# moddyz/stereo-to-multiview-cuda

Hardware: AMD Instinct MI355X
Metric: stereo->8-view frames/sec @1080p d=64; cost-agg HBM GB/s vs roofline (higher is better)
Workload: dtype f32; 1 GPU; 1920x1080 synthetic stereo frame, D=64, zd=32, full stereo->8-view frame: cost init + cross aggregation + WTA + DCC/IRV x5/bilateral + 6 DIBR views + interlacing, one frame per GPU per step; stages=3, usd=34, lsd=17, views=8, aggregation=matrix pipe (stm_kernels_aggm.hip)

## Files before the change

### include/stm_hip.h

```cpp
#ifndef STM_HIP_H
#define STM_HIP_H

#ifdef __cplusplus
extern "C" {
#endif
#if defined(STM_BUILD) && defined(__GNUC__)
#pragma GCC visibility push(default)
#endif

int         stm_version(void);
void        stm_set_stream(void *hip_stream);
void       *stm_get_stream(void);
void        stm_set_error_mode(int mode);
const char *stm_last_error(void);
void        stm_release_workspace(void);
void        stm_prof_enable(int on);
void        stm_prof_reset(void);
int         stm_prof_read(const char *kernel, float *total_ms);
void        stm_set_agg_variant(int v);
int         stm_agg_path(int num_disp, int zero_disp, int num_rows, int num_cols, int usd, int stages);
int         stm_first_pass_path(int num_disp, int zero_disp, int num_rows, int num_cols, int usd, int stages);
int         stm_px_order(int num_disp, int zero_disp, int num_rows, int num_cols, int usd, int stages);
void        stm_set_irv_paper_ratio(int on);
int         stm_set_irv_chunk(int entries);
int         stm_irv_path(int num_rows, int num_cols, int usd, int iterations, int device_flavour, int with_dcc);
int         stm_set_lens(int mode, double pitch, double slope, double centre);
int         stm_set_depth(int mode, float gain, float conv);
int         stm_set_depth_auto(float disp_lo, float disp_hi, float max_gain, int clip_permille, float rate, float *d_state);
int         stm_set_antialias(int mode, float strength, int max_radius, float gate);
void        stm_get_antialias(int out_mode[2], float out[2]);
int         stm_set_align(int mode, float a, float b, float c);
int         stm_set_align_auto(int radius, float rate, float *d_state);
void        stm_get_align(int out_mode[2], float out[4]);
int         stm_set_balance(int mode, const unsigned char *lut768);
int         stm_set_balance_auto(int max_shift, float rate, int *d_state);
void        stm_get_balance(int out_mode[2], float *out_rate, unsigned char out_lut[768]);
int         stm_set_cut(int mode, int thresh_permille, int min_gap, int *d_state);
void        stm_get_cut(int out[3]);
int         stm_set_active(int mode, const int rect[4], int fill, float fill_disp);
int         stm_set_active_auto(int thresh_luma, int lit_permille, int max_bar_permille, int hold, int *d_state);
void        stm_get_active(int out[10], float *fill_disp);
int         stm_set_layout(int layout, int tiles_x, int tiles_y, int order, int filter);
void        stm_get_layout(int *out);
int         stm_set_output(int format, int matrix, int pitch, int uv_row);
void        stm_get_output(int out[4]);
int         stm_set_overlay(int mode, const unsigned char *d_overlay, int ov_rows, int ov_cols, int x0, int y0, float disparity);
void        stm_get_overlay(int out[5], float *disparity);
int         stm_set_overlay_auto(int mode, int near_permille, float margin, int pad, float limit_lo, float limit_hi, float rate_near,
// ... 43 lines not shown
void stm_d_dr_irv(float *d_disp, unsigned char *d_outliers, unsigned char **d_cross, int thresh_s, float thresh_h,
                  int num_rows, int num_cols, int num_disp, int zero_disp, int usd, int iterations);
void stm_dr_interp(float *disp, unsigned char *outliers, unsigned char *img, int num_rows, int num_cols, int elem_sz);
void stm_d_dr_interp(float *d_disp, unsigned char *d_outliers, unsigned char *d_img, int num_rows, int num_cols, int elem_sz);
void stm_filter_bilateral_1(float *img, int radius, float sigma_color, float sigma_spatial,
                            int num_rows, int num_cols, int num_disp);
void stm_d_filter_bilateral_1(float *d_img, int radius, float sigma_color, float sigma_spatial,
                              int num_rows, int num_cols, int num_disp);
void stm_filter_gaussian_1(float *img, int radius, float sigma_spatial, int num_rows, int num_cols);
void stm_d_filter_gaussian_1(float *d_img, int radius, float sigma_spatial, int num_rows, int num_cols);
void stm_filter_bleed_1(unsigned char *img, int radius, int num_rows, int num_cols);
void stm_d_filter_bleed_1(unsigned char *d_img, int radius, int num_rows, int num_cols);
void stm_filter_median(float *img, int num_rows, int num_cols);
void stm_d_filter_median(float *d_img, int num_rows, int num_cols);

void stm_dibr_occl(unsigned char *occl_l, unsigned char *occl_r, float *disp_l, float *disp_r,
                   int num_rows, int num_cols);
void stm_d_dibr_occl(unsigned char *d_occl_l, unsigned char *d_occl_r, float *d_disp_l, float *d_disp_r,
                     int num_rows, int num_cols);
void stm_dibr_occl_to_mask(float *mask_l, float *mask_r, unsigned char *occl_l, unsigned char *occl_r,
                           int num_rows, int num_cols);
void stm_d_dibr_occl_to_mask(float *d_mask_l, float *d_mask_r, unsigned char *d_occl_l, unsigned char *d_occl_r,
                             int num_rows, int num_cols);
void stm_dibr_dbm(unsigned char *img_out, unsigned char *img_in_l, unsigned char *img_in_r,
                  float *disp_l, float *disp_r, unsigned char *occl_l, unsigned char *occl_r,
                  float *mask_l, float *mask_r, float shift, int num_rows, int num_cols, int elem_sz);
void stm_d_dibr_dbm(unsigned char *d_img_out, unsigned char *d_img_in_l, unsigned char *d_img_in_r,
                    float *d_disp_l, float *d_disp_r, unsigned char *d_occl_l, unsigned char *d_occl_r,
                    float *d_mask_l, float *d_mask_r, float shift, int num_rows, int num_cols, int elem_sz);
void stm_dibr_dbm_lin(unsigned char *img_out, unsigned char *img_in_l, unsigned char *img_in_r,
                      float *disp_l, float *disp_r, unsigned char *occl_l, unsigned char *occl_r,
                      float *mask_l, float *mask_r, float shift, int num_rows, int num_cols, int elem_sz);
void stm_d_dibr_dbm_lin(unsigned char *d_img_out, unsigned char *d_img_in_l, unsigned char *d_img_in_r,
                        float *d_disp_l, float *d_disp_r, unsigned char *d_occl_l, unsigned char *d_occl_r,
                        float *d_mask_l, float *d_mask_r, float shift, int num_rows, int num_cols, int elem_sz);
void stm_dibr_dfm(unsigned char *img_out, unsigned char *img_in_l, unsigned char *img_in_r,
                  float *disp_l, float *disp_r, float shift, int num_rows, int num_cols, int elem_sz);
void stm_d_dibr_dfm(unsigned char *d_img_out, unsigned char *d_img_in_l, unsigned char *d_img_in_r,
                    float *d_disp_l, float *d_disp_r, float shift, int num_rows, int num_cols, int elem_sz);

void stm_mux_multiview(unsigned char **views, unsigned char *out_data, int num_views, float angle,
                       int in_rows, int in_cols, int out_rows, int out_cols, int elem_sz);
void stm_d_mux_multiview(unsigned char **d_views, unsigned char *d_out_data, int num_views, float angle,
                         int in_rows, int in_cols, int out_rows, int out_cols, int elem_sz);
void stm_mux_multiview_lens(unsigned char **views, unsigned char *out_data, int num_views, int mode, double pitch, double slope,
                            double centre, int in_rows, int in_cols, int out_rows, int out_cols, int elem_sz);
// ... 231 lines not shown
```

### stereo-to-multiview-cuda_amd/_lib.py

```python
import ctypes as C
import os

HERE = os.path.dirname(os.path.abspath(__file__))
LIB_PATH = os.path.join(HERE, "libstm_hip.so")
if os.environ.get("STM_LIB") == "timing":
    LIB_PATH = os.path.join(HERE, "libstm_hip_timing.so")

u8p = C.POINTER(C.c_uint8)
f32p = C.POINTER(C.c_float)
u32p = C.POINTER(C.c_uint32)
u8pp = C.POINTER(u8p)
f32pp = C.POINTER(f32p)
vp = C.c_void_p
i, f, d = C.c_int, C.c_float, C.c_double

PROTOS = {
    "stm_version": ([], i),
    "stm_set_stream": ([vp], None),
    "stm_get_stream": ([], vp),
    "stm_set_error_mode": ([i], None),
    "stm_last_error": ([], C.c_char_p),
    "stm_release_workspace": ([], None),
    "stm_prof_enable": ([i], None),
    "stm_prof_reset": ([], None),
    "stm_prof_read": ([C.c_char_p, f32p], i),
    "stm_set_agg_variant": ([i], None),
    "stm_agg_path": ([i, i, i, i, i, i], i),
    "stm_first_pass_path": ([i, i, i, i, i, i], i),
    "stm_px_order": ([i, i, i, i, i, i], i),
    "stm_set_irv_paper_ratio": ([i], None),
    "stm_set_irv_chunk": ([i], i),
    "stm_irv_path": ([i, i, i, i, i, i], i),
    "stm_set_ref_quirks": ([i], None),
    "stm_set_lens": ([i, d, d, d], i),
    "stm_set_layout": ([i, i, i, i, i], i),
    "stm_get_layout": ([C.POINTER(C.c_int)], None),
    "stm_set_output": ([i, i, i, i], i),
    "stm_get_output": ([C.POINTER(C.c_int)], None),
    "stm_set_overlay": ([i, vp, i, i, i, i, f], i),
    "stm_get_overlay": ([C.POINTER(C.c_int), f32p], None),
    "stm_set_overlay_auto": ([i, i, f, i, f, f, f, f, vp], i),
    "stm_get_overlay_auto": ([C.POINTER(C.c_int), f32p], None),
    "stm_set_quilt_lds_limit": ([i], None),
    "stm_set_packing": ([i, i, i, i], i),
    "stm_get_packing": ([C.POINTER(C.c_int)], None),
    "stm_set_depth": ([i, f, f], i),
    "stm_set_depth_auto": ([f, f, f, i, f, vp], i),
    "stm_set_antialias": ([i, f, i, f], i),
    "stm_get_antialias": ([C.POINTER(C.c_int), f32p], None),
    "stm_set_align": ([i, f, f, f], i),
    "stm_set_align_auto": ([i, f, vp], i),
    "stm_get_align": ([C.POINTER(C.c_int), f32p], None),
    "stm_set_balance": ([i, u8p], i),
    "stm_set_balance_auto": ([i, f, vp], i),
    "stm_get_balance": ([C.POINTER(C.c_int), f32p, u8p], None),
# ... 11 lines not shown
    "stm_dc_subpixel": ([f32pp, f32p, i, i, i, i], None),
    "stm_d_dc_subpixel": ([vp, vp, i, i, i, i], None),
    "stm_dc_hslo": ([f32pp, f32p, u8p, u8p, f, f, f, i, i, i, i, i], None),
    "stm_d_dc_hslo": ([vp, vp, vp, vp, f, f, f, i, i, i, i, i], None),
    "stm_dr_dcc": ([u8p, u8p, f32p, f32p, i, i], None),
    "stm_d_dr_dcc": ([vp, vp, vp, vp, i, i], None),
    "stm_dr_irv": ([f32p, u8p, u8pp, i, f, i, i, i, i, i, i], None),
    "stm_d_dr_irv": ([vp, vp, vp, i, f, i, i, i, i, i, i], None),
    "stm_dr_interp": ([f32p, u8p, u8p, i, i, i], None),
    "stm_d_dr_interp": ([vp, vp, vp, i, i, i], None),
    "stm_filter_bilateral_1": ([f32p, i, f, f, i, i, i], None),
    "stm_d_filter_bilateral_1": ([vp, i, f, f, i, i, i], None),
    "stm_filter_gaussian_1": ([f32p, i, f, i, i], None),
    "stm_d_filter_gaussian_1": ([vp, i, f, i, i], None),
    "stm_filter_bleed_1": ([u8p, i, i, i], None),
    "stm_d_filter_bleed_1": ([vp, i, i, i], None),
    "stm_filter_median": ([f32p, i, i], None),
    "stm_generate_gaussian_kernel": ([f32p, i, f], None),
    "stm_d_filter_median": ([vp, i, i], None),
    "stm_dibr_occl": ([u8p, u8p, f32p, f32p, i, i], None),
    "stm_d_dibr_occl": ([vp, vp, vp, vp, i, i], None),
    "stm_dibr_occl_to_mask": ([f32p, f32p, u8p, u8p, i, i], None),
    "stm_d_dibr_occl_to_mask": ([vp, vp, vp, vp, i, i], None),
    "stm_dibr_dbm": ([u8p, u8p, u8p, f32p, f32p, u8p, u8p, f32p, f32p, f, i, i, i], None),
    "stm_d_dibr_dbm": ([vp, vp, vp, vp, vp, vp, vp, vp, vp, f, i, i, i], None),
    "stm_dibr_dbm_lin": ([u8p, u8p, u8p, f32p, f32p, u8p, u8p, f32p, f32p, f, i, i, i], None),
    "stm_d_dibr_dbm_lin": ([vp, vp, vp, vp, vp, vp, vp, vp, vp, f, i, i, i], None),
    "stm_dibr_dfm": ([u8p, u8p, u8p, f32p, f32p, f, i, i, i], None),
    "stm_d_dibr_dfm": ([vp, vp, vp, vp, vp, f, i, i, i], None),
    "stm_mux_multiview": ([u8pp, u8p, i, f, i, i, i, i, i], None),
    "stm_d_mux_multiview": ([vp, vp, i, f, i, i, i, i, i], None),
    "stm_mux_multiview_lens": ([u8pp, u8p, i, i, d, d, d, i, i, i, i, i], None),
    "stm_d_mux_multiview_lens": ([vp, vp, i, i, d, d, d, i, i, i, i, i], None),
    "stm_quilt_multiview": ([u8pp, u8p, i, i, i, i, i, i, i, i, i, i], None),
    "stm_d_quilt_multiview": ([vp, vp, i, i, i, i, i, i, i, i, i, i], None),
    "stm_mux_overlay": ([u8p, u8p, i, i, i, i, f, i, f, i, d, d, d, i, i, i, i, i, i, i], None),
    "stm_d_mux_overlay": ([vp, vp, i, i, i, i, f, i, f, i, d, d, d, i, i, i, i, i, i, i], None),
    "stm_d_demux_sbs": ([vp, vp, vp, i, i, i, i], None),
    "stm_demux_nv12": ([u8p, u8p, u8p, i, u8p, i, i, i, i, i, i], None),
    "stm_d_demux_nv12": ([vp, vp, vp, i, vp, i, i, i, i, i, i], None),
    "stm_mux_nv12": ([u8p, i, u8p, i, u8p, i, i, i, i], None),
    "stm_d_mux_nv12": ([vp, i, vp, i, vp, i, i, i, i], None),
    "stm_demux_packed": ([u8p, u8p, u8p, i, i, i, i, i, i, i, i], None),
    "stm_d_demux_packed": ([vp, vp, vp, i, i, i, i, i, i, i, i], None),
    "stm_demux_nv12_packed": ([u8p, u8p, u8p, i, u8p, i, i, i, i, i, i, i, i, i, i], None),
    "stm_d_demux_nv12_packed": ([vp, vp, vp, i, vp, i, i, i, i, i, i, i, i, i, i], None),
# ... 101 lines not shown
```

### stereo-to-multiview-cuda_amd/csrc/stm_api.hip

```cpp
#include "stm_common.h"
#include <initializer_list>
#include <mutex>
#include "../../include/stm_hip.h"

#include <map>
#include <stdio.h>
#include <stdlib.h>
#include <string.h>
#include <tuple>
#include <vector>

using namespace stm;

namespace {

struct DevTable {
    float *d = nullptr;
    size_t n = 0;
};
std::map<std::tuple<int, int, float, float>, DevTable> g_tables;

int cur_dev()
{
    int dev = 0;
// ... 154 lines not shown
Arms arms_from_table(unsigned char **d_cross)
{
    u8 *h[4];
    STM_CHECK(hipMemcpyAsync(h, d_cross, sizeof h, hipMemcpyDeviceToHost, stream()));
    sync();
    return Arms{h[0], h[1], h[2], h[3]};
}

void core_bilateral(float *d_img, int radius, float sigma_color, float sigma_spatial, int H, int W, int D)
{
    size_t HW = (size_t)H * W;
    float *tmp = Workspace::get<float>(HW);
    launch_bilateral(d_img, tmp, gauss2d_table(radius, sigma_spatial), gauss1d_table(D, sigma_color), radius, H, W, D);
    STM_CHECK(hipMemcpyAsync(d_img, tmp, HW * sizeof(float), hipMemcpyDeviceToDevice, stream()));
}

void core_dbm(u8 *d_out, const u8 *d_l, const u8 *d_r, const float *disp_l, const float *disp_r, const float *mask_l,
              const float *mask_r, float shift, int H, int W, int elem_sz, int g_radius, float g_sigma, bool linear = false)
{
    size_t HW = (size_t)H * W;
    float *blend = Workspace::get<float>(HW);
    launch_gaussian_max(mask_r, blend, gauss2d_table(g_radius, g_sigma), g_radius, g_sigma, H, W, true);
    launch_view_synth(d_out, d_l, d_r, disp_l, disp_r, mask_l, mask_r, blend, shift, H, W, elem_sz, linear);
}

void dbm_device(const char *fn, unsigned char *d_img_out, unsigned char *d_img_in_l, unsigned char *d_img_in_r, float *d_disp_l,
                float *d_disp_r, float *d_mask_l, float *d_mask_r, float shift, int num_rows, int num_cols, int elem_sz, bool linear)
{
    if (!args_ok(fn, {{"num_rows", num_rows, 1}, {"num_cols", num_cols, 1}, {"elem_sz", elem_sz, 3}})) return;
    Workspace::begin((size_t)num_rows * num_cols * 4 + 1024);
    if (elem_sz > 3)
        STM_CHECK(hipMemsetAsync(d_img_out, 0, (size_t)num_rows * num_cols * elem_sz, stream()));
    core_dbm(d_img_out, d_img_in_l, d_img_in_r, d_disp_l, d_disp_r, d_mask_l, d_mask_r, shift, num_rows, num_cols, elem_sz,
             10, 15.0f, linear);
}
void dbm_host(const char *fn, unsigned char *img_out, unsigned char *img_in_l, unsigned char *img_in_r, float *disp_l, float *disp_r,
              float *mask_l, float *mask_r, float shift, int num_rows, int num_cols, int elem_sz, bool linear)
{
    if (!args_ok(fn, {{"num_rows", num_rows, 1}, {"num_cols", num_cols, 1}, {"elem_sz", elem_sz, 3}})) return;
    size_t HW = (size_t)num_rows * num_cols;
    Workspace::begin(3 * HW * elem_sz + 20 * HW + 8192);
    u8 *l = up(img_in_l, HW * elem_sz), *r = up(img_in_r, HW * elem_sz), *o = Workspace::get<u8>(HW * elem_sz);
    float *dl = up(disp_l, HW), *dr = up(disp_r, HW), *ml = up(mask_l, HW), *mr = up(mask_r, HW);
    STM_CHECK(hipMemsetAsync(o, 0, HW * elem_sz, stream()));
    core_dbm(o, l, r, dl, dr, ml, mr, shift, num_rows, num_cols, elem_sz, 7, 10.0f, linear);
    down(img_out, o, HW * elem_sz);
// ... 527 lines not shown
                     int num_cols)
{
    if (!args_ok("d_dibr_occl", {{"num_rows", num_rows, 1}, {"num_cols", num_cols, 1}})) return;
    launch_occl(d_occl_l, d_occl_r, d_disp_l, d_disp_r, num_rows, num_cols);
}
void stm_dibr_occl(unsigned char *occl_l, unsigned char *occl_r, float *disp_l, float *disp_r, int num_rows, int num_cols)
{
    if (!args_ok("dibr_occl", {{"num_rows", num_rows, 1}, {"num_cols", num_cols, 1}})) return;
    size_t HW = (size_t)num_rows * num_cols;
    Workspace::begin(10 * HW + 4096);
    float *dl = up(disp_l, HW), *dr = up(disp_r, HW);
    u8 *ol = Workspace::get<u8>(HW), *orr = Workspace::get<u8>(HW);
    launch_occl(ol, orr, dl, dr, num_rows, num_cols);
    down(occl_l, ol, HW); down(occl_r, orr, HW);
    sync();
}

void stm_d_dibr_occl_to_mask(float *d_mask_l, float *d_mask_r, unsigned char *d_occl_l, unsigned char *d_occl_r,
                             int num_rows, int num_cols)
{
    if (!args_ok("d_dibr_occl_to_mask", {{"num_rows", num_rows, 1}, {"num_cols", num_cols, 1}})) return;
    launch_occl_to_mask(d_mask_l, d_mask_r, d_occl_l, d_occl_r, num_rows, num_cols);
}
void stm_dibr_occl_to_mask(float *mask_l, float *mask_r, unsigned char *occl_l, unsigned char *occl_r, int num_rows,
                           int num_cols)
{
    if (!args_ok("dibr_occl_to_mask", {{"num_rows", num_rows, 1}, {"num_cols", num_cols, 1}})) return;
    size_t HW = (size_t)num_rows * num_cols;
    Workspace::begin(10 * HW + 4096);
    u8 *ol = up(occl_l, HW), *orr = up(occl_r, HW);
    float *ml = Workspace::get<float>(HW), *mr = Workspace::get<float>(HW);
    launch_occl_to_mask(ml, mr, ol, orr, num_rows, num_cols);
    down(mask_l, ml, HW); down(mask_r, mr, HW);
    sync();
}

void stm_d_dibr_dbm(unsigned char *d_img_out, unsigned char *d_img_in_l, unsigned char *d_img_in_r, float *d_disp_l,
                    float *d_disp_r, unsigned char *d_occl_l, unsigned char *d_occl_r, float *d_mask_l, float *d_mask_r,
                    float shift, int num_rows, int num_cols, int elem_sz)
{
    (void)d_occl_l; (void)d_occl_r;
    dbm_device("d_dibr_dbm", d_img_out, d_img_in_l, d_img_in_r, d_disp_l, d_disp_r, d_mask_l, d_mask_r, shift, num_rows, num_cols,
               elem_sz, false);
}
void stm_dibr_dbm(unsigned char *img_out, unsigned char *img_in_l, unsigned char *img_in_r, float *disp_l, float *disp_r,
                  unsigned char *occl_l, unsigned char *occl_r, float *mask_l, float *mask_r, float shift, int num_rows,
// ... 1061 lines not shown
        if (!overlay_tiles_ok(fn, lo, num_views)) return false;
        if (overlay_auto().mode == 1 && !overlay_fit_size_ok(fn, a.num_rows, a.num_cols)) return false;
    }
    if (lo.layout == 0) return frame_output_ok(fn, lo, Hout, Wout);
    if (lens().mode != 0) {
        char msg[200];
        snprintf(msg, sizeof msg, "%s: layout 1 (quilt) together with lens mode %d: a quilt is not interlaced, set one of them to 0", fn, lens().mode);
        fail(msg, "layout, lens", __FILE__, __LINE__);
        return false;
    }
    return quilt_args_ok(fn, lo, num_views, a.num_rows, a.num_cols, Hout, Wout, "num_views", "num_rows_out", "num_cols_out") &&
           frame_output_ok(fn, lo, Hout, Wout);
}

void frame_render(u8 *img_l, u8 *img_r, float *d_disp_l, float *d_disp_r, u8 *d_interlaced, const FrameArgs &a, float **depth_state_out,
                  const int *d_rect)
{
    *depth_state_out = nullptr;
    const int H = a.num_rows, W = a.num_cols, Hout = a.num_rows_out, Wout = a.num_cols_out, elem_sz = a.elem_sz, N = a.num_views;
    const float angle = a.angle;
    const bool linear = (a.stages & 0x800) != 0;
    const size_t HW = (size_t)H * W, IMG = HW * elem_sz;
    float *mask_l = Workspace::get<float>(HW), *mask_r = Workspace::get<float>(HW), *blend = Workspace::get<float>(HW);
    launch_hitmask_rows(mask_l, mask_r, d_disp_l, d_disp_r, H, W);
    launch_gaussian_max(mask_r, blend, gauss2d_table(10, 15.0f), 10, 15.0f, H, W, true);

    const Lens ln = lens();
    const Depth dp = depth();
    const Layout lo = layout();
    float inv_y = 0.0f;
    int ymod = 1;
    if (lo.layout == 0 && dp.mode != 0 && ln.mode == 0 && !mux_geom_ok(N, angle, elem_sz, nullptr, &inv_y, &ymod)) return;
    float *state = nullptr;
    if (dp.mode == 2) {
        uint32_t *hist = Workspace::get<uint32_t>(4096);
        state = dp.d_state ? dp.d_state : Workspace::get<float>(4);
        launch_depth_fit(state, hist, d_disp_l, d_disp_r, H, W, dp.disp_lo, dp.disp_hi, dp.max_gain, dp.clip_permille, dp.rate,
                         dp.d_state == nullptr, d_rect);
        *depth_state_out = state;
    }
    const Antialias aa = antialias();
    if (aa.mode == 1) {
        u8 *flt[2] = {Workspace::get<u8>(IMG), Workspace::get<u8>(IMG)};
        const u8 *src[2] = {img_l, img_r};
        const float *dsp[2] = {d_disp_l, d_disp_r};
        launch_view_prefilter(2, flt, src, dsp, H, W, elem_sz, N, aa.strength, aa.max_radius, aa.gate, dp.mode == 1 ? dp.gain : 1.0f,
                              dp.mode == 1 ? dp.conv : 0.0f, state);
        img_l = flt[0];
// ... 814 lines not shown
```

### stereo-to-multiview-cuda_amd/csrc/stm_common.h

```cpp
#pragma once
#include <hip/hip_runtime.h>
#include <stddef.h>
#include <stdint.h>

typedef unsigned char u8;

namespace stm {

void fail(const char *what, const char *expr, const char *file, int line);
bool failed();
void clear_failed();
struct ApiNest { ApiNest(); ~ApiNest(); };
bool api_outermost();
void release_host_frame_bufs();
bool nv12_args_ok(const char *fn, int num_rows, int num_cols_sbs, int num_cols, const char *cols_name, int pitch_y, int pitch_uv, int matrix);
#define STM_CHECK(expr)                                                                  \
    do {                                                                                 \
        hipError_t _e = (expr);                                                          \
        if (_e != hipSuccess) ::stm::fail(hipGetErrorString(_e), #expr, __FILE__, __LINE__); \
    } while (0)
#define STM_CHECK_LAUNCH() STM_CHECK(hipGetLastError())
#define STM_LAUNCH(...)                                     \
    do {                                                    \
        if (!::stm::failed()) hipLaunchKernelGGL(__VA_ARGS__); \
// ... 183 lines not shown
void launch_dcc(u8 *out_l, u8 *out_r, const float *disp_l, const float *disp_r, u8 *hit_l, u8 *hit_r, int H, int W);
void launch_irv(int nviews, float *const *disp, u8 *const *outl, const u8 *const *up, const u8 *const *down,
                const u8 *const *left, const u8 *const *right, int thresh_s, float thresh_h,
                int H, int W, int D, int zd, int usd, int iterations, bool device_flavour, bool with_dcc = false);
int irv_path(int H, int W, int usd, int iterations, bool device_flavour, bool with_dcc);
void launch_bilateral(const float *in, float *out, const float *spatial, const float *color,
                      int radius, int H, int W, int D);
void launch_bilateral2(const float *in_a, float *out_a, const float *in_b, float *out_b, const float *spatial, const float *color,
                       int radius, int H, int W, int D, bool integer_maps = false, const float *one_value = nullptr, int zd = 0);
void launch_gaussian_max(const float *in, float *out, const float *spatial, int radius, float sigma, int H, int W,
                         bool invert_input);
void launch_subpix(Vol cost, float *disp, int D, int zd, int H, int W);
void launch_subpix_frame(float *const *pq, float *const *quads, float *const *disp, const u8 *const *armL, const u8 *const *armR, int D,
                         int zd, int H, int W);
void launch_interp(int nviews, float *const *disp, const u8 *const *outl, const u8 *const *img, int H, int W, int elem_sz);
void launch_demux_sbs(u8 *l, u8 *r, const u8 *sbs, int H, int Wsbs, int W, int elem_sz);
void launch_demux_sbs_packed(u8 *l, u8 *r, uint32_t *pk_l, uint32_t *pk_r, uint32_t *wide_l, uint32_t *wide_r, const u8 *sbs, int H,
                             int Wsbs, int W, int elem_sz);
void launch_occl(u8 *occl_l, u8 *occl_r, const float *disp_l, const float *disp_r, int H, int W);
void launch_bleed(const u8 *in, u8 *out, int radius, int H, int W);
void launch_median3(const float *in, float *out, int H, int W);
void launch_dcc_rows(u8 *out_l, u8 *out_r, const float *disp_l, const float *disp_r, int H, int W);
void launch_hitmask_rows(float *mask_l, float *mask_r, const float *disp_l, const float *disp_r, int H, int W);
void launch_occl_to_mask(float *mask_l, float *mask_r, const u8 *occl_l, const u8 *occl_r, int H, int W);
void launch_view_synth(u8 *out, const u8 *img_l, const u8 *img_r, const float *disp_l, const float *disp_r,
                       const float *mask_l, const float *mask_r, const float *blend, float shift, int H, int W, int elem_sz,
                       bool linear = false);
void launch_view_synth_all(u8 *views, size_t view_stride, int N, const u8 *img_l, const u8 *img_r, const float *disp_l,
                           const float *disp_r, const float *mask_l, const float *mask_r, const float *blend, int H, int W,
                           int elem_sz, bool linear = false);
void launch_fwarp(u8 *out, const u8 *img, const float *disp, float shift, unsigned long long *keys, int H, int W, int elem_sz);
void launch_scale_bilinear(const u8 *in, u8 *out, int in_rows, int in_cols, int out_rows, int out_cols, int elem_sz);
void launch_disp_scale(float *out, const float *in, int out_rows, int out_cols, int in_rows, int in_cols, float disp_scale);
void launch_view_table(u8 **tab, u8 *first, u8 *last, u8 *mem, size_t stride, int N);
void launch_disp_upsample(int nviews, float *const *out, const float *const *dlow, const u8 *const *ilow, const u8 *const *img,
                          const float *tab, int H, int W, int h, int w, int elem_sz, float up);
void launch_disp_temporal(int nviews, float *const *cur, const float *const *prev, const u8 *const *img, const u8 *const *img_prev,
                          const size_t *byte_off, int H, int W, int stride, int elem_sz, float alpha, int thresh_color, float thresh_disp);
void launch_synth_mux(const u8 *img_l, const u8 *img_r, const float *disp_l, const float *disp_r, const float *mask_l, const float *mask_r,
                      const float *blend, u8 *out, int N, float y_interval, float inv_y_interval, int ymod, int Hin, int Win, int Hout,
                      int Wout, int elem_sz, int variant, bool linear = false);
void launch_mux(const u8 *const *d_views, u8 *out, int N, float y_interval, float inv_y_interval, int ymod,
                int Hin, int Win, int Hout, int Wout, int elem_sz, int variant);
void launch_mux_lens(const u8 *const *d_views, u8 *out, int N, const Lens &ln, int Hin, int Win, int Hout, int Wout, int elem_sz);
void launch_synth_mux_lens(const u8 *img_l, const u8 *img_r, const float *disp_l, const float *disp_r, const float *mask_l,
                           const float *mask_r, const float *blend, u8 *out, int N, const Lens &ln, int Hin, int Win, int Hout, int Wout,
// ... 172 lines not shown
```

### stereo-to-multiview-cuda_amd/csrc/stm_kernels_dibr.hip

```cpp
#include "stm_common.h"
#include "stm_views.h"

namespace stm {

__global__ __launch_bounds__(256) void stm_k_demux_sbs(u8 *__restrict__ l, u8 *__restrict__ r, const u8 *__restrict__ sbs,
                                                       int H, int Wsbs, int W, int elem_sz)
{
    int x = blockIdx.x * 256 + threadIdx.x, y = blockIdx.y;
    if (x >= Wsbs) return;
    const u8 *s = sbs + ((size_t)y * Wsbs + x) * elem_sz;
    u8 *d;
    if (x < W) d = l + ((size_t)y * W + x) * elem_sz;
    else if (x - W < W) d = r + ((size_t)y * W + (x - W)) * elem_sz;
    else return;
    d[0] = s[0]; d[1] = s[1]; d[2] = s[2];
}
__global__ __launch_bounds__(256) void stm_k_demux_sbs_packed(u8 *__restrict__ l, u8 *__restrict__ r, uint32_t *__restrict__ pk_l,
                                                              uint32_t *__restrict__ pk_r, uint32_t *__restrict__ wide_l,
                                                              uint32_t *__restrict__ wide_r, const u8 *__restrict__ sbs, int Wsbs,
                                                              int W, int elem_sz)
{
    const int x = blockIdx.x * 256 + threadIdx.x, y = blockIdx.y;
    if (x >= 2 * W) return;
    const u8 *s = sbs + ((size_t)y * Wsbs + x) * elem_sz;
// ... 142 lines not shown
    __syncthreads();
    const size_t orow = (size_t)ty * W;
    for (int tx = threadIdx.x; tx < W; tx += 256) {
        int cnt_l = 0, cnt_r = 0;
#pragma unroll
        for (int j = 0; j < 3; ++j) {
            const u8 *ol = hm_lds + (size_t)j * 2 * W, *orr = ol + W;
#pragma unroll
            for (int x = -1; x <= 1; ++x) {
                int sx = tx + x;
                if (sx < 0) sx = -sx;
                if (sx > W - 1) sx = W - 1 - x;
                sx = min(max(sx, 0), W - 1);
                cnt_l += ol[sx] > 0;
                cnt_r += orr[sx] > 0;
            }
        }
        const u8 vl = ((double)cnt_l > 8 * 0.30) ? (u8)1 : hm_lds[2 * W + tx];
        const u8 vr = ((double)cnt_r > 8 * 0.30) ? (u8)1 : hm_lds[3 * W + tx];
        mask_l[orow + tx] = vl == 1 ? 1.0f : 0.0f;
        mask_r[orow + tx] = vr == 1 ? 1.0f : 0.0f;
    }
}
void launch_hitmask_rows(float *mask_l, float *mask_r, const float *disp_l, const float *disp_r, int H, int W)
{
    const size_t smem = 6 * (size_t)W;
    if (smem > 64 * 1024) STM_CHECK(hipFuncSetAttribute((const void *)stm_k_hitmask_rows, hipFuncAttributeMaxDynamicSharedMemorySize, (int)smem));
    STM_LAUNCH(stm_k_hitmask_rows, dim3(H), dim3(256), smem, stream(), mask_l, mask_r, disp_l, disp_r, H, W);
    STM_CHECK_LAUNCH();
}

template <bool LINEAR>
__device__ __forceinline__ u8 warp_tap(const u8 *__restrict__ img, size_t row, float fx, int c, int W, int elem_sz)
{
    if constexpr (!LINEAR) {
        const int sx = (int)fx;
        return img[(row + sx) * elem_sz + c];
    } else {
        const int x0 = (int)floorf(fx);
        const int x1 = min(x0 + 1, W - 1);
        const float wx = fx - (float)x0;
        const float a = (float)img[(row + x0) * elem_sz + c] * (1.0f - wx);
        const float b = (float)img[(row + x1) * elem_sz + c] * wx;
        const float top = a + b;
        return (u8)top;
    }
}
template <bool LINEAR>
__global__ __launch_bounds__(256) void stm_k_view_synth(u8 *__restrict__ out, const u8 *__restrict__ img_l,
                                                        const u8 *__restrict__ img_r, const float *__restrict__ disp_l,
                                                        const float *__restrict__ disp_r, const float *__restrict__ mask_l,
// ... 275 lines not shown
    ta = top * (1.0f - wy);
    tb = bot * wy;
    return (u8)(ta + tb);
}
template <bool LINEAR>
__global__ __launch_bounds__(256) void stm_k_synth_mux(SynthArgs a, u8 *__restrict__ out, int N, float y_interval, float inv_y, int ymod,
                                                       int Hin, int Win, int Hout, int Wout, int elem_sz, int variant)
{
    const int tx = blockIdx.x * 256 + threadIdx.x, ty = blockIdx.y;
    if (tx >= Wout) return;
    float xs = ((float)tx / (float)Wout) * (float)Win;
    xs = fminf(fmaxf(xs, 0.0f), (float)(Win - 1));
    float ys = ((float)ty / (float)Hout) * (float)Hin;
    ys = fminf(fmaxf(ys, 0.0f), (float)(Hin - 1));
    const int r_view = mux_r_view(tx, ty, N, y_interval, inv_y, ymod, variant);
    int g_view = r_view + 1, b_view = r_view + 2;
    if (g_view >= N) g_view -= N;
    if (b_view >= N) b_view -= N;
    const size_t o = ((size_t)tx + (size_t)ty * Wout) * elem_sz;
    out[o + 0] = synth_bilinear<LINEAR>(a, N, b_view, 0, xs, ys, Win, Hin, elem_sz);
    out[o + 1] = synth_bilinear<LINEAR>(a, N, g_view, 1, xs, ys, Win, Hin, elem_sz);
    out[o + 2] = synth_bilinear<LINEAR>(a, N, r_view, 2, xs, ys, Win, Hin, elem_sz);
}
void launch_synth_mux(const u8 *img_l, const u8 *img_r, const float *disp_l, const float *disp_r, const float *mask_l, const float *mask_r,
                      const float *blend, u8 *out, int N, float y_interval, float inv_y_interval, int ymod, int Hin, int Win, int Hout,
                      int Wout, int elem_sz, int variant, bool linear)
{
    SynthArgs a{img_l, img_r, disp_l, disp_r, mask_l, mask_r, blend};
    ProfScope p("synth_mux");
    if (linear)
        STM_LAUNCH(stm_k_synth_mux<true>, dim3(cdiv(Wout, 256), Hout), dim3(256), 0, stream(), a, out, N, y_interval, inv_y_interval,
                   ymod, Hin, Win, Hout, Wout, elem_sz, variant);
    else
        STM_LAUNCH(stm_k_synth_mux<false>, dim3(cdiv(Wout, 256), Hout), dim3(256), 0, stream(), a, out, N, y_interval, inv_y_interval,
                   ymod, Hin, Win, Hout, Wout, elem_sz, variant);
    STM_CHECK_LAUNCH();
}

void launch_mux(const u8 *const *d_views, u8 *out, int N, float y_interval, float inv_y_interval, int ymod, int Hin,
                int Win, int Hout, int Wout, int elem_sz, int variant)
{
    ProfScope p("mux");
    STM_LAUNCH(stm_k_mux, dim3(cdiv(Wout, 256), Hout), dim3(256), 0, stream(), d_views, out, N, y_interval,
                       inv_y_interval, ymod, Hin, Win, Hout, Wout, elem_sz, variant);
    STM_CHECK_LAUNCH();
}

template <int MODE>
__global__ __launch_bounds__(256) void stm_k_mux_lens(const u8 *const *__restrict__ views, u8 *__restrict__ out, int N, Lens g, int Hin,
                                                      int Win, int Hout, int Wout, int elem_sz)
{
    const int tx = blockIdx.x * 256 + threadIdx.x, ty = blockIdx.y;
// ... 115 lines not shown
        n10 = lens_nb(a, x0, y1, Win);
        if (wx != 0.0f) n11 = lens_nb(a, x1, y1, Win);
    }
    const size_t o = ((size_t)tx + (size_t)ty * Wout) * elem_sz;
#pragma unroll
    for (int c = 0; c < 3; ++c) {
        int v;
        float w, shift;
        lens_pick<MODE>(lens_phase(tx, ty, c, g), N, v, w, shift);
        if constexpr (MODE == 3) {
            out[o + c] = lens_bilinear<LINEAR, true>(a, n00, n01, n10, n11, wx, wy, N, 0, shift, c, Win, elem_sz);
        } else {
            const u8 A = lens_bilinear<LINEAR, false>(a, n00, n01, n10, n11, wx, wy, N, v, 0.0f, c, Win, elem_sz);
            if constexpr (MODE == 1) {
                out[o + c] = A;
            } else {
                const u8 B = lens_bilinear<LINEAR, false>(a, n00, n01, n10, n11, wx, wy, N, v + 1, 0.0f, c, Win, elem_sz);
                const float p = (float)A * (1.0f - w);
                const float q = (float)B * w;
                out[o + c] = (u8)(p + q);
            }
        }
    }
}
template <int MODE>
static void launch_synth_mux_lens_mode(const SynthArgs &a, u8 *out, int N, const Lens &ln, int Hin, int Win, int Hout, int Wout,
                                       int elem_sz, bool linear)
{
    if (linear)
        STM_LAUNCH((stm_k_synth_mux_lens<MODE, true>), dim3(cdiv(Wout, 256), Hout), dim3(256), 0, stream(), a, out, N, ln, Hin, Win, Hout,
                   Wout, elem_sz);
    else
        STM_LAUNCH((stm_k_synth_mux_lens<MODE, false>), dim3(cdiv(Wout, 256), Hout), dim3(256), 0, stream(), a, out, N, ln, Hin, Win, Hout,
                   Wout, elem_sz);
}
void launch_synth_mux_lens(const u8 *img_l, const u8 *img_r, const float *disp_l, const float *disp_r, const float *mask_l,
                           const float *mask_r, const float *blend, u8 *out, int N, const Lens &ln, int Hin, int Win, int Hout, int Wout,
                           int elem_sz, bool linear)
{
    SynthArgs a{img_l, img_r, disp_l, disp_r, mask_l, mask_r, blend};
    ProfScope p("synth_mux");
    if (ln.mode == 1) launch_synth_mux_lens_mode<1>(a, out, N, ln, Hin, Win, Hout, Wout, elem_sz, linear);
    else if (ln.mode == 2) launch_synth_mux_lens_mode<2>(a, out, N, ln, Hin, Win, Hout, Wout, elem_sz, linear);
    else launch_synth_mux_lens_mode<3>(a, out, N, ln, Hin, Win, Hout, Wout, elem_sz, linear);
    STM_CHECK_LAUNCH();
}
// ... 716 lines not shown
```

### stereo-to-multiview-cuda_amd/csrc/stm_runtime.hip

```cpp
#include "stm_common.h"
#include "../../include/stm_hip.h"

#include <float.h>
#include <math.h>
#include <cmath>
#include <stdio.h>
#include <stdlib.h>
#include <string.h>
#include <mutex>
#include <string>
#include <vector>

namespace stm {

static int g_error_mode = 0;
static thread_local std::string g_last_error;
static thread_local bool g_failed = false;
bool failed() { return g_failed; }
void clear_failed() { g_failed = false; }
static thread_local int g_api_depth = 0;
ApiNest::ApiNest() { ++g_api_depth; }
ApiNest::~ApiNest() { --g_api_depth; }
bool api_outermost() { return g_api_depth == 0; }

// ... 781 lines not shown
        ++n;
    }
    if (total_ms) *total_ms = tot;
    return n;
}
void stm_set_ref_quirks(int on) { stm::g_ref_quirks = on ? 1 : 0; }
void stm_set_irv_paper_ratio(int on) { stm::g_irv_paper_ratio = on ? 1 : 0; }
int stm_set_irv_chunk(int entries)
{
    if (stm::api_outermost()) stm::clear_failed();
    if (entries < 0 || entries > 16) {
        char msg[120];
        snprintf(msg, sizeof msg, "set_irv_chunk: entries = %d, must be 0 (the library's own rule) or 1 .. 16", entries);
        stm::fail(msg, "entries", __FILE__, __LINE__);
        return -1;
    }
    stm::g_irv_chunk = entries;
    return 0;
}
int stm_irv_path(int num_rows, int num_cols, int usd, int iterations, int device_flavour, int with_dcc)
{
    return stm::irv_path(num_rows, num_cols, usd, iterations, device_flavour != 0, with_dcc != 0);
}
int stm_set_lens(int mode, double pitch, double slope, double centre)
{
    if (stm::api_outermost()) stm::clear_failed();
    if (!stm::lens_params_ok("set_lens", mode, 0, 3, pitch, slope, centre)) return -1;
    stm::set_lens(mode == 0 ? stm::Lens{0, 0.0, 0.0, 0.0} : stm::Lens{mode, pitch, slope, centre});
    return 0;
}
int stm_set_layout(int layout, int tiles_x, int tiles_y, int order, int filter)
{
    if (stm::api_outermost()) stm::clear_failed();
    if (!stm::layout_params_ok("set_layout", layout, tiles_x, tiles_y, order, filter)) return -1;
    stm::set_layout(layout == 0 ? stm::Layout{0, 1, 1, 0, 0} : stm::Layout{layout, tiles_x, tiles_y, order, filter});
    return 0;
}
void stm_get_layout(int *out)
{
    const stm::Layout lo = stm::layout();
    out[0] = lo.layout; out[1] = lo.tiles_x; out[2] = lo.tiles_y; out[3] = lo.order; out[4] = lo.filter;
}
int stm_set_output(int format, int matrix, int pitch, int uv_row)
{
    if (stm::api_outermost()) stm::clear_failed();
    if (!stm::output_params_ok("set_output", format, matrix, pitch, uv_row)) return -1;
// ... 225 lines not shown
```

### stereo-to-multiview-cuda_amd/device_api.py

```python
import ctypes as C

import torch

from ._lib import f32p, f32pp, lib


def _use_current_stream():
    lib().stm_set_stream(C.c_void_p(torch.cuda.current_stream().cuda_stream))


def _p(t):
    return C.c_void_p(t.data_ptr())


STAGE_SUBPIXEL = 0x200
STAGE_INTERP = 0x400
STAGE_LINEAR_WARP = 0x800
STAGE_GUIDED_UP = 0x1000
STAGE_TEMPORAL = 0x2000
TEMPORAL_DEFAULTS = (0.5, 24, 1.5)


class FrameParams:

# ... 3 lines not shown
        self.ad_coeff, self.census_coeff = ad_coeff, census_coeff
        self.ucd, self.lcd, self.usd, self.lsd = ucd, lcd, usd, lsd
        self.thresh_s, self.thresh_h = thresh_s, thresh_h
        self.out_rows, self.out_cols = out_rows, out_cols


AGG_MATRIX_PIPE, AGG_PX, AGG_VREGS, AGG_HREGS, AGG_SPLIT = 1, 2, 4, 8, 1 << 16


def agg_path(num_disp, zero_disp, num_rows, num_cols, usd, stages=3):
    return int(lib().stm_agg_path(int(num_disp), int(zero_disp), int(num_rows), int(num_cols), int(usd), int(stages)))


def agg_path_waves(path):
    return (int(path) >> 8) & 0xff


def first_pass_path(num_disp, zero_disp, num_rows, num_cols, usd, stages=3):
    return int(lib().stm_first_pass_path(int(num_disp), int(zero_disp), int(num_rows), int(num_cols), int(usd), int(stages)))


def px_order(num_disp, zero_disp, num_rows, num_cols, usd, stages=3):
    return int(lib().stm_px_order(int(num_disp), int(zero_disp), int(num_rows), int(num_cols), int(usd), int(stages)))


IRV_PRUNE, IRV_RUNS, IRV_CHAIN = 1, 2, 4


def irv_path(num_rows, num_cols, usd, iterations=5, device_flavour=True, with_dcc=False):
    return int(lib().stm_irv_path(int(num_rows), int(num_cols), int(usd), int(iterations), int(bool(device_flavour)), int(bool(with_dcc))))


def irv_path_tile_sh(path):
    return (int(path) >> 8) & 0xf


def irv_path_chunk(path):
    return (int(path) >> 16) & 0x1f


def set_irv_chunk(entries=0):
    if int(lib().stm_set_irv_chunk(int(entries))) != 0:
        raise ValueError("stm_set_irv_chunk(%d) refused: %s" % (entries, lib().stm_last_error().decode()))


def set_lens(mode, pitch=0.0, slope=0.0, centre=0.0):
# ... 717 lines not shown
```

Before: 683.1 frames/s.

## Band hitmask rows per block and load lens neighbours once in synth mux

Replaces the one-row-per-block hitmask kernel with a banded version in which each block scatters B+2 disparity rows into shared memory once and computes B output rows, so the halo rows are not re-scattered by neighbouring blocks. Adds a synth_mux kernel that fetches the four bilinear lens neighbours once per pixel and reuses them for all three colour channels, where the old kernel sampled them separately per channel. Both paths are on by default and can be disabled through an agg_variant digit. It also exposes a tail_path query and a frame_masks entry point. The banded kernel uses more shared memory per block and runs fewer blocks.

```diff
diff --git a/include/stm_hip.h b/include/stm_hip.h
--- a/include/stm_hip.h
+++ b/include/stm_hip.h
@@ -24,6 +24,7 @@
 void        stm_set_irv_paper_ratio(int on);
 int         stm_set_irv_chunk(int entries);
 int         stm_irv_path(int num_rows, int num_cols, int usd, int iterations, int device_flavour, int with_dcc);
+int         stm_tail_path(int num_rows, int num_cols);
 int         stm_set_lens(int mode, double pitch, double slope, double centre);
 int         stm_set_depth(int mode, float gain, float conv);
 int         stm_set_depth_auto(float disp_lo, float disp_hi, float max_gain, int clip_permille, float rate, float *d_state);
@@ -113,6 +114,8 @@
                            int num_rows, int num_cols);
 void stm_d_dibr_occl_to_mask(float *d_mask_l, float *d_mask_r, unsigned char *d_occl_l, unsigned char *d_occl_r,
                              int num_rows, int num_cols);
+void stm_d_dibr_frame_masks(float *d_mask_l, float *d_mask_r, float *d_blend, float *d_disp_l, float *d_disp_r, int num_rows,
+                            int num_cols);
 void stm_dibr_dbm(unsigned char *img_out, unsigned char *img_in_l, unsigned char *img_in_r,
                   float *disp_l, float *disp_r, unsigned char *occl_l, unsigned char *occl_r,
                   float *mask_l, float *mask_r, float shift, int num_rows, int num_cols, int elem_sz);
diff --git a/stereo-to-multiview-cuda_amd/_lib.py b/stereo-to-multiview-cuda_amd/_lib.py
--- a/stereo-to-multiview-cuda_amd/_lib.py
+++ b/stereo-to-multiview-cuda_amd/_lib.py
@@ -31,6 +31,7 @@
     "stm_set_irv_paper_ratio": ([i], None),
     "stm_set_irv_chunk": ([i], i),
     "stm_irv_path": ([i, i, i, i, i, i], i),
+    "stm_tail_path": ([i, i], i),
     "stm_set_ref_quirks": ([i], None),
     "stm_set_lens": ([i, d, d, d], i),
     "stm_set_layout": ([i, i, i, i, i], i),
@@ -88,6 +89,7 @@
     "stm_d_dibr_occl": ([vp, vp, vp, vp, i, i], None),
     "stm_dibr_occl_to_mask": ([f32p, f32p, u8p, u8p, i, i], None),
     "stm_d_dibr_occl_to_mask": ([vp, vp, vp, vp, i, i], None),
+    "stm_d_dibr_frame_masks": ([vp, vp, vp, vp, vp, i, i], None),
     "stm_dibr_dbm": ([u8p, u8p, u8p, f32p, f32p, u8p, u8p, f32p, f32p, f, i, i, i], None),
     "stm_d_dibr_dbm": ([vp, vp, vp, vp, vp, vp, vp, vp, vp, f, i, i, i], None),
     "stm_dibr_dbm_lin": ([u8p, u8p, u8p, f32p, f32p, u8p, u8p, f32p, f32p, f, i, i, i], None),
diff --git a/stereo-to-multiview-cuda_amd/csrc/stm_api.hip b/stereo-to-multiview-cuda_amd/csrc/stm_api.hip
--- a/stereo-to-multiview-cuda_amd/csrc/stm_api.hip
+++ b/stereo-to-multiview-cuda_amd/csrc/stm_api.hip
@@ -200,6 +200,12 @@
     float *blend = Workspace::get<float>(HW);
     launch_gaussian_max(mask_r, blend, gauss2d_table(g_radius, g_sigma), g_radius, g_sigma, H, W, true);
     launch_view_synth(d_out, d_l, d_r, disp_l, disp_r, mask_l, mask_r, blend, shift, H, W, elem_sz, linear);
+}
+
+void core_frame_masks(float *mask_l, float *mask_r, float *blend, const float *d_disp_l, const float *d_disp_r, int H, int W)
+{
+    launch_hitmask_rows(mask_l, mask_r, d_disp_l, d_disp_r, H, W);
+    launch_gaussian_max(mask_r, blend, gauss2d_table(10, 15.0f), 10, 15.0f, H, W, true);
 }
 
 void dbm_device(const char *fn, unsigned char *d_img_out, unsigned char *d_img_in_l, unsigned char *d_img_in_r, float *d_disp_l,
@@ -773,6 +779,11 @@
     if (!args_ok("d_dibr_occl_to_mask", {{"num_rows", num_rows, 1}, {"num_cols", num_cols, 1}})) return;
     launch_occl_to_mask(d_mask_l, d_mask_r, d_occl_l, d_occl_r, num_rows, num_cols);
 }
+void stm_d_dibr_frame_masks(float *d_mask_l, float *d_mask_r, float *d_blend, float *d_disp_l, float *d_disp_r, int num_rows, int num_cols)
+{
+    if (!args_ok("d_dibr_frame_masks", {{"num_rows", num_rows, 1}, {"num_cols", num_cols, 1}})) return;
+    core_frame_masks(d_mask_l, d_mask_r, d_blend, d_disp_l, d_disp_r, num_rows, num_cols);
+}
 void stm_dibr_occl_to_mask(float *mask_l, float *mask_r, unsigned char *occl_l, unsigned char *occl_r, int num_rows,
                            int num_cols)
 {
@@ -1880,8 +1891,7 @@
     const bool linear = (a.stages & 0x800) != 0;
     const size_t HW = (size_t)H * W, IMG = HW * elem_sz;
     float *mask_l = Workspace::get<float>(HW), *mask_r = Workspace::get<float>(HW), *blend = Workspace::get<float>(HW);
-    launch_hitmask_rows(mask_l, mask_r, d_disp_l, d_disp_r, H, W);
-    launch_gaussian_max(mask_r, blend, gauss2d_table(10, 15.0f), 10, 15.0f, H, W, true);
+    core_frame_masks(mask_l, mask_r, blend, d_disp_l, d_disp_r, H, W);
 
     const Lens ln = lens();
     const Depth dp = depth();
diff --git a/stereo-to-multiview-cuda_amd/csrc/stm_common.h b/stereo-to-multiview-cuda_amd/csrc/stm_common.h
--- a/stereo-to-multiview-cuda_amd/csrc/stm_common.h
+++ b/stereo-to-multiview-cuda_amd/csrc/stm_common.h
@@ -229,6 +229,8 @@
 void launch_median3(const float *in, float *out, int H, int W);
 void launch_dcc_rows(u8 *out_l, u8 *out_r, const float *disp_l, const float *disp_r, int H, int W);
 void launch_hitmask_rows(float *mask_l, float *mask_r, const float *disp_l, const float *disp_r, int H, int W);
+int hitmask_band(int H, int W);
+int tail_path(int H, int W);
 void launch_occl_to_mask(float *mask_l, float *mask_r, const u8 *occl_l, const u8 *occl_r, int H, int W);
 void launch_view_synth(u8 *out, const u8 *img_l, const u8 *img_r, const float *disp_l, const float *disp_r,
                        const float *mask_l, const float *mask_r, const float *blend, float shift, int H, int W, int elem_sz,
diff --git a/stereo-to-multiview-cuda_amd/csrc/stm_kernels_dibr.hip b/stereo-to-multiview-cuda_amd/csrc/stm_kernels_dibr.hip
--- a/stereo-to-multiview-cuda_amd/csrc/stm_kernels_dibr.hip
+++ b/stereo-to-multiview-cuda_amd/csrc/stm_kernels_dibr.hip
@@ -188,11 +188,93 @@
         mask_r[orow + tx] = vr == 1 ? 1.0f : 0.0f;
     }
 }
+constexpr int HM_BAND = 2, HM_T = 512;
+template <int B>
+__global__ __launch_bounds__(HM_T) void stm_k_hitmask_bands(float *__restrict__ mask_l, float *__restrict__ mask_r,
+                                                            const float *__restrict__ disp_l, const float *__restrict__ disp_r,
+                                                            int H, int W, int WP)
+{
+    extern __shared__ u8 hm_lds[];
+    const int y0 = blockIdx.x * B;
+    uint32_t *lds32 = (uint32_t *)hm_lds;
+    for (int i = threadIdx.x; i < (B + 2) * 2 * WP / 4; i += HM_T) lds32[i] = 0;
+    __syncthreads();
+#pragma unroll
+    for (int k = 0; k < B + 2; ++k) {
+        const int r = y0 - 1 + k;
+        if (r < 0 || r >= H) continue;
+        u8 *ol = hm_lds + (size_t)k * 2 * WP, *orr = ol + WP;
+        const size_t row = (size_t)r * W;
+        for (int x = threadIdx.x; x < W; x += HM_T) {
+            int sd = (int)(disp_l[row + x] * 1.0f);
+            orr[min(max(x + sd, 0), W - 1)] = 1;
+            sd = (int)(disp_r[row + x] * -1.0f);
+            ol[min(max(x + sd, 0), W - 1)] = 1;
+        }
+    }
+    __syncthreads();
+    for (int tx = threadIdx.x; tx < W; tx += HM_T) {
+        int sxs[3];
+#pragma unroll
+        for (int x = -1; x <= 1; ++x) {
+            int sx = tx + x;
+            if (sx < 0) sx = -sx;
+            if (sx > W - 1) sx = W - 1 - x;
+            sxs[x + 1] = min(max(sx, 0), W - 1);
+        }
+#pragma unroll
+        for (int r = 0; r < B; ++r) {
+            const int ty = y0 + r;
+            if (ty >= H) break;
+            int cnt_l = 0, cnt_r = 0;
+#pragma unroll
+            for (int j = 0; j < 3; ++j) {
+                const int y = j - 1;
+                int sy = ty + y;
+                if (sy < 0) sy = -sy;
+                if (sy > H - 1) sy = H - 1 - y;
+                sy = min(max(sy, 0), H - 1);
+                const u8 *ol = hm_lds + (size_t)(sy - (y0 - 1)) * 2 * WP, *orr = ol + WP;
+#pragma unroll
+                for (int x = 0; x < 3; ++x) {
+                    cnt_l += ol[sxs[x]] > 0;
+                    cnt_r += orr[sxs[x]] > 0;
+                }
+            }
+            const u8 *cl = hm_lds + (size_t)(r + 1) * 2 * WP;
+            const u8 vl = ((double)cnt_l > 8 * 0.30) ? (u8)1 : cl[tx];
+            const u8 vr = ((double)cnt_r > 8 * 0.30) ? (u8)1 : cl[WP + tx];
+            const size_t o = (size_t)ty * W + tx;
+            mask_l[o] = vl == 1 ? 1.0f : 0.0f;
+            mask_r[o] = vr == 1 ? 1.0f : 0.0f;
+        }
+    }
+}
+int hitmask_band(int H, int W)
+{
+    if ((agg_variant() / 100) % 10 == 8) return 0;
+    const size_t smem = (size_t)(HM_BAND + 2) * 2 * ((W + 3) & ~3);
+    return smem <= 128 * 1024 ? HM_BAND : 0;
+}
+bool synth_mux_loads_once();
+int tail_path(int H, int W)
+{
+    const int band = hitmask_band(H, W);
+    return (band != 0 ? 1 | band << 8 : 0) | (synth_mux_loads_once() ? 2 : 0);
+}
 void launch_hitmask_rows(float *mask_l, float *mask_r, const float *disp_l, const float *disp_r, int H, int W)
 {
-    const size_t smem = 6 * (size_t)W;
-    if (smem > 64 * 1024) STM_CHECK(hipFuncSetAttribute((const void *)stm_k_hitmask_rows, hipFuncAttributeMaxDynamicSharedMemorySize, (int)smem));
-    STM_LAUNCH(stm_k_hitmask_rows, dim3(H), dim3(256), smem, stream(), mask_l, mask_r, disp_l, disp_r, H, W);
+    if (hitmask_band(H, W) == 0) {
+        const size_t smem = 6 * (size_t)W;
+        if (smem > 64 * 1024) STM_CHECK(hipFuncSetAttribute((const void *)stm_k_hitmask_rows, hipFuncAttributeMaxDynamicSharedMemorySize, (int)smem));
+        STM_LAUNCH(stm_k_hitmask_rows, dim3(H), dim3(256), smem, stream(), mask_l, mask_r, disp_l, disp_r, H, W);
+        STM_CHECK_LAUNCH();
+        return;
+    }
+    const int WP = (W + 3) & ~3;
+    const size_t smem = (size_t)(HM_BAND + 2) * 2 * WP;
+    if (smem > 64 * 1024) STM_CHECK(hipFuncSetAttribute((const void *)stm_k_hitmask_bands<HM_BAND>, hipFuncAttributeMaxDynamicSharedMemorySize, (int)smem));
+    STM_LAUNCH(stm_k_hitmask_bands<HM_BAND>, dim3(cdiv(H, HM_BAND)), dim3(HM_T), smem, stream(), mask_l, mask_r, disp_l, disp_r, H, W, WP);
     STM_CHECK_LAUNCH();
 }
 
@@ -514,12 +596,19 @@
     out[o + 1] = synth_bilinear<LINEAR>(a, N, g_view, 1, xs, ys, Win, Hin, elem_sz);
     out[o + 2] = synth_bilinear<LINEAR>(a, N, r_view, 2, xs, ys, Win, Hin, elem_sz);
 }
+static void launch_synth_mux_nb(const SynthArgs &a, u8 *out, int N, float y_interval, float inv_y_interval, int ymod, int Hin, int Win, int Hout,
+                                int Wout, int elem_sz, int variant, bool linear);
+bool synth_mux_loads_once() { return (agg_variant() / 100) % 10 != 8; }
 void launch_synth_mux(const u8 *img_l, const u8 *img_r, const float *disp_l, const float *disp_r, const float *mask_l, const float *mask_r,
                       const float *blend, u8 *out, int N, float y_interval, float inv_y_interval, int ymod, int Hin, int Win, int Hout,
                       int Wout, int elem_sz, int variant, bool linear)
 {
     SynthArgs a{img_l, img_r, disp_l, disp_r, mask_l, mask_r, blend};
     ProfScope p("synth_mux");
+    if (synth_mux_loads_once()) {
+        launch_synth_mux_nb(a, out, N, y_interval, inv_y_interval, ymod, Hin, Win, Hout, Wout, elem_sz, variant, linear);
+        return;
+    }
     if (linear)
         STM_LAUNCH(stm_k_synth_mux<true>, dim3(cdiv(Wout, 256), Hout), dim3(256), 0, stream(), a, out, N, y_interval, inv_y_interval,
                    ymod, Hin, Win, Hout, Wout, elem_sz, variant);
@@ -681,6 +770,46 @@
             }
         }
     }
+}
+template <bool LINEAR>
+__global__ __launch_bounds__(256) void stm_k_synth_mux_nb(SynthArgs a, u8 *__restrict__ out, int N, float y_interval, float inv_y, int ymod,
+                                                          int Hin, int Win, int Hout, int Wout, int elem_sz, int variant)
+{
+    const int tx = blockIdx.x * 256 + threadIdx.x, ty = blockIdx.y;
+    if (tx >= Wout) return;
+    float xs = ((float)tx / (float)Wout) * (float)Win;
+    xs = fminf(fmaxf(xs, 0.0f), (float)(Win - 1));
+    float ys = ((float)ty / (float)Hout) * (float)Hin;
+    ys = fminf(fmaxf(ys, 0.0f), (float)(Hin - 1));
+    const int r_view = mux_r_view(tx, ty, N, y_interval, inv_y, ymod, variant);
+    int g_view = r_view + 1, b_view = r_view + 2;
+    if (g_view >= N) g_view -= N;
+    if (b_view >= N) b_view -= N;
+    const int x0 = (int)floorf(xs), y0 = (int)floorf(ys);
+    const int x1 = min(x0 + 1, Win - 1), y1 = min(y0 + 1, Hin - 1);
+    const float wx = xs - (float)x0, wy = ys - (float)y0;
+    const LensNb n00 = lens_nb(a, x0, y0, Win);
+    LensNb n01 = n00, n10 = n00, n11 = n00;
+    if (wx != 0.0f) n01 = lens_nb(a, x1, y0, Win);
+    if (wy != 0.0f) {
+        n10 = lens_nb(a, x0, y1, Win);
+        if (wx != 0.0f) n11 = lens_nb(a, x1, y1, Win);
+    }
+    const size_t o = ((size_t)tx + (size_t)ty * Wout) * elem_sz;
+    out[o + 0] = lens_bilinear<LINEAR, false>(a, n00, n01, n10, n11, wx, wy, N, b_view, 0.0f, 0, Win, elem_sz);
+    out[o + 1] = lens_bilinear<LINEAR, false>(a, n00, n01, n10, n11, wx, wy, N, g_view, 0.0f, 1, Win, elem_sz);
+    out[o + 2] = lens_bilinear<LINEAR, false>(a, n00, n01, n10, n11, wx, wy, N, r_view, 0.0f, 2, Win, elem_sz);
+}
+static void launch_synth_mux_nb(const SynthArgs &a, u8 *out, int N, float y_interval, float inv_y_interval, int ymod, int Hin, int Win, int Hout,
+                                int Wout, int elem_sz, int variant, bool linear)
+{
+    if (linear)
+        STM_LAUNCH(stm_k_synth_mux_nb<true>, dim3(cdiv(Wout, 256), Hout), dim3(256), 0, stream(), a, out, N, y_interval, inv_y_interval, ymod,
+                   Hin, Win, Hout, Wout, elem_sz, variant);
+    else
+        STM_LAUNCH(stm_k_synth_mux_nb<false>, dim3(cdiv(Wout, 256), Hout), dim3(256), 0, stream(), a, out, N, y_interval, inv_y_interval, ymod,
+                   Hin, Win, Hout, Wout, elem_sz, variant);
+    STM_CHECK_LAUNCH();
 }
 template <int MODE>
 static void launch_synth_mux_lens_mode(const SynthArgs &a, u8 *out, int N, const Lens &ln, int Hin, int Win, int Hout, int Wout,
diff --git a/stereo-to-multiview-cuda_amd/csrc/stm_runtime.hip b/stereo-to-multiview-cuda_amd/csrc/stm_runtime.hip
--- a/stereo-to-multiview-cuda_amd/csrc/stm_runtime.hip
+++ b/stereo-to-multiview-cuda_amd/csrc/stm_runtime.hip
@@ -827,6 +827,7 @@
 {
     return stm::irv_path(num_rows, num_cols, usd, iterations, device_flavour != 0, with_dcc != 0);
 }
+int stm_tail_path(int num_rows, int num_cols) { return stm::tail_path(num_rows, num_cols); }
 int stm_set_lens(int mode, double pitch, double slope, double centre)
 {
     if (stm::api_outermost()) stm::clear_failed();
diff --git a/stereo-to-multiview-cuda_amd/device_api.py b/stereo-to-multiview-cuda_amd/device_api.py
--- a/stereo-to-multiview-cuda_amd/device_api.py
+++ b/stereo-to-multiview-cuda_amd/device_api.py
@@ -49,6 +49,13 @@
 
 def px_order(num_disp, zero_disp, num_rows, num_cols, usd, stages=3):
     return int(lib().stm_px_order(int(num_disp), int(zero_disp), int(num_rows), int(num_cols), int(usd), int(stages)))
+
+
+TAIL_BANDS, TAIL_LOADS_ONCE = 1, 2
+
+
+def tail_path(num_rows, num_cols):
+    return int(lib().stm_tail_path(int(num_rows), int(num_cols)))
 
 
 IRV_PRUNE, IRV_RUNS, IRV_CHAIN = 1, 2, 4
```

After: 687.6 frames/s (median of 6 runs). About the same (+0.7%).
